# VladimirP1/rs-sync

Hardware: NVIDIA B200
Metric: presync_loss_evals_per_s (higher is better)
Workload: dtype f64

## Files before the change

### rs-sync_b200/csrc/engine.cu

```cuda
#include "engine.h"

#include <algorithm>
#include <atomic>
#include <cmath>
#include <cstdio>
#include <map>
#include <mutex>
#include <tuple>
#include <utility>
#include <vector>

#include "device_math.cuh"
#include "gyro_scan.h"

namespace rs {

namespace {

constexpr unsigned FULL = 0xffffffffu;

#ifdef RS_CHECKED
__device__ int* g_assert_slot = nullptr;
#define RS_ASSERT(cond)                                                      \
    do {                                                                     \
// ... 288 lines not shown
    return Vec3{M[0], M[1], M[2]};
}

template <int SLOTS>
__device__ __noinline__ unsigned long long warp_exact_quartile(const WarpSmem& w, int n, int lane,
                                                               double vx, double vy, double vz) {
    constexpr int NP = SLOTS * 32;
    const unsigned long long nanbits = 0x7ff8000000000000ULL;
    double r2[SLOTS];
    unsigned h[SLOTS];
    __syncwarp();
#pragma unroll
    for (int s = 0; s < SLOTS; ++s) {
        const int i = s * 32 + lane;
        const double p0 = w.P[i], p1 = w.P[NP + i], p2 = w.P[2 * NP + i];
        const double inv = (i < n) ? row_inv_norm(p0, p1, p2) : __longlong_as_double((long long)nanbits);
        const double r = dot3(p0 * inv, p1 * inv, p2 * inv, vx, vy, vz);
        r2[s] = r * r;
        h[s] = (unsigned)__double2hiint(r2[s]) & 0x7fffffffu;
    }
    const int kth = n / 4;
    int cl, ce;
    const unsigned H = warp_select_hi<SLOTS>(h, kth, 0x7ff80000u, lane, cl, ce);
    int rem = kth - cl;
    unsigned cur = 0u, lo_ans = 0u;
    for (;;) {
        unsigned mn = 0xffffffffu, c = 0u;
#pragma unroll
        for (int s = 0; s < SLOTS; ++s) {
            const unsigned lo = (unsigned)__double2loint(r2[s]);
            if (h[s] == H && lo >= cur) mn = min(mn, lo);
        }
        mn = __reduce_min_sync(FULL, mn);
#pragma unroll
        for (int s = 0; s < SLOTS; ++s)
            c += (h[s] == H && (unsigned)__double2loint(r2[s]) == mn) ? 1u : 0u;
        c = __reduce_add_sync(FULL, c);
        if (rem < (int)c) { lo_ans = mn; break; }
        rem -= (int)c;
        cur = mn + 1u;
    }
    return ((unsigned long long)H << 32) | lo_ans;
}

constexpr float kMargin = 1.4e-6f;

__device__ __forceinline__ unsigned up_bits(unsigned qbits) {
    const float u = __fadd_ru(__fsqrt_ru(__uint_as_float(qbits)), kMargin);
    return __float_as_uint(__fmul_ru(u, u));
}
__device__ __forceinline__ float sqrt_approx(float x) {
    float y;
    asm("sqrt.approx.ftz.f32 %0, %1;" : "=f"(y) : "f"(x));
    return y;
}

template <int SLOTS>
__device__ __forceinline__ int warp_count_le(const float (&s)[SLOTS], unsigned pv) {
    const float nt = -__uint_as_float(pv + 1u);
    unsigned c = 0;
#pragma unroll
    for (int i = 0; i < SLOTS; ++i) c += __float_as_uint(s[i] + nt) >> 31;
    return (int)__reduce_add_sync(FULL, c);
}
template <int SLOTS>
__device__ __forceinline__ unsigned warp_min_ge(const float (&s)[SLOTS], unsigned lo) {
    unsigned mn = 0xffffffffu;
#pragma unroll
    for (int i = 0; i < SLOTS; ++i) mn = min(mn, __float_as_uint(s[i]) - lo);
    return lo + __reduce_min_sync(FULL, mn);
}
template <int SLOTS>
__device__ __forceinline__ unsigned warp_max_lt(const float (&s)[SLOTS], unsigned hi_excl) {
    unsigned mn = 0xffffffffu;
    const unsigned top = hi_excl - 1u;
#pragma unroll
    for (int i = 0; i < SLOTS; ++i) mn = min(mn, top - __float_as_uint(s[i]));
    return top - __reduce_min_sync(FULL, mn);
}

template <int SLOTS>
__device__ __forceinline__ unsigned warp_select32(const float (&s)[SLOTS], int kk, unsigned hi_excl,
                                                  int chi, int npad, int n, bool sample) {
    unsigned lo = 0u;
    int clo = 0, poor = 0;
    for (int round = 0;; ++round) {
        RS_ASSERT(round < 80 && clo <= kk && kk < chi && lo < hi_excl);
        if (hi_excl - lo == 1u) return lo;
        if (kk == clo) return warp_min_ge<SLOTS>(s, lo);
        if (kk == chi - 1) return warp_max_lt<SLOTS>(s, hi_excl);
        unsigned pv;
        if (sample) {
            sample = false;
            const int js = min((32 * (kk - npad)) / n, 31);
            const unsigned k0 = __float_as_uint(s[0]);
            unsigned cur = 0u;
            pv = 0u;
            for (int i = 0; i <= js; ++i) {
                pv = cur + __reduce_min_sync(FULL, k0 - cur);
                cur = pv + 1u;
            }
        } else if (poor >= 2) {
            poor = 0;
            pv = lo + ((hi_excl - lo) >> 1);
        } else {
            const int cl = (lo == 0u) ? npad : clo;
            const float frac = ((float)(kk - cl) + 0.5f) / (float)(chi - cl);
            const float sl = sqrt_approx(__uint_as_float(lo));
            const float sh = sqrt_approx(__uint_as_float(hi_excl));
            const float sq = fmaf(sh - sl, frac, sl);
            pv = __float_as_uint(sq * sq);
        }
        pv = max(pv, lo);
        pv = min(pv, hi_excl - 2u);
        const int cnt = warp_count_le<SLOTS>(s, pv);
        if (cnt > kk) {
            poor = (2 * (cnt - clo) > (chi - clo)) ? poor + 1 : 0;
            hi_excl = pv + 1u;
            chi = cnt;
        } else {
            poor = (2 * (chi - cnt) > (chi - clo)) ? poor + 1 : 0;
            lo = pv + 1u;
            clo = cnt;
        }
    }
}

template <int SLOTS>
__device__ __forceinline__ bool load_normalised_rows32(const double* __restrict__ sP, int n, int lane,
                                                       float (&nx)[SLOTS], float (&ny)[SLOTS],
                                                       float (&nz)[SLOTS]) {
    constexpr int NP = SLOTS * 32;
    float fin = 0.f;
#pragma unroll
    for (int s = 0; s < SLOTS; ++s) {
        const int i = s * 32 + lane;
        const double r0 = sP[i], r1 = sP[NP + i], r2 = sP[2 * NP + i];
        const float n2 = (float)dot3(r0, r1, r2, r0, r1, r2);
        float rs;
        asm("rsqrt.approx.f32 %0, %1;" : "=f"(rs) : "f"(n2));
        if (i >= n) rs = 0.f;
        else if (n2 <= 1e-24f) rs = __uint_as_float(0x7fc00000u);
        nx[s] = (float)r0 * rs;
        ny[s] = (float)r1 * rs;
        nz[s] = (float)r2 * rs;
        fin += (fabsf(nx[s]) + fabsf(ny[s])) + fabsf(nz[s]);
    }
    return __all_sync(FULL, (__float_as_uint(fin) & 0x7f800000u) != 0x7f800000u);
}

enum FastStatus { kFastOk = 0, kFastUndecided = 1, kFastRowsNotFinite = 2, kFastRetry = 3 };

template <int SLOTS>
__device__ __forceinline__ FastStatus warp_ransac_fast(const DeviceData& dd, const FrameDesc& fd,
                                                       const WarpSmem& w, int iters, uint64_t key,
                                                       int lane, double M[3], int* settled,
                                                       unsigned prior, unsigned* tau_out) {
    constexpr int NP = SLOTS * 32;
    float nx[SLOTS], ny[SLOTS], nz[SLOTS];
    if (!load_normalised_rows32<SLOTS>(w.P, fd.n, lane, nx, ny, nz)) return kFastRowsNotFinite;
    const int n = fd.n;
    const int npad = NP - n;
    const int kk = n / 4 + npad;
    unsigned tau = 0x7f800000u;
    float nthr = 0.f;
    unsigned thr1 = 0u;
    bool has_real = true;
    if (prior) {
        tau = thr1 = prior;
        nthr = -__uint_as_float(prior);
        has_real = false;
    }
    M[0] = M[1] = M[2] = 0.0;
    float* hyp = w.hyp;
    for (int j0 = 0; j0 < iters; j0 += 32) {
        double v[3] = {0.0, 0.0, 0.0};
        if (j0 + lane < iters) draw_hypothesis(dd, fd, w.P, NP, key, (uint32_t)(j0 + lane), v);
        __syncwarp();
        hyp[lane] = (float)v[0];
        hyp[32 + lane] = (float)v[1];
        hyp[64 + lane] = (float)v[2];
        __syncwarp();
        const int cnt = (iters - j0) < 32 ? (iters - j0) : 32;
        int t = 0;
        while (t < cnt) {
            float sq[SLOTS];
            int tc, chi;
            unsigned hi_excl;
            bool first = false;
            if (tau == 0x7f800000u) {
                const float vx = hyp[t], vy = hyp[32 + t], vz = hyp[64 + t];
                unsigned mx = 0u;
#pragma unroll
                for (int s = 0; s < SLOTS; ++s) {
                    const float r = fmaf(nz[s], vz, fmaf(ny[s], vy, nx[s] * vx));
                    sq[s] = r * r;
                    mx = max(mx, __float_as_uint(sq[s]));
                }
                mx = __reduce_max_sync(FULL, mx);
                if (mx >= 0x7f800000u) return kFastUndecided;
                hi_excl = mx + 1u;
                chi = NP;
                tc = t;
                first = true;
                t += 1;
            } else {
                const int t1 = (t + 1 < cnt) ? t + 1 : t;
                const float2 vx2 = make_float2(hyp[t], hyp[t1]);
                const float2 vy2 = make_float2(hyp[32 + t], hyp[32 + t1]);
                const float2 vz2 = make_float2(hyp[64 + t], hyp[64 + t1]);
                const float2 nt2 = make_float2(nthr, nthr);
                float2 rr[SLOTS];
                unsigned c0 = 0, c1 = 0;
#pragma unroll
                for (int s = 0; s < SLOTS; ++s) {
                    float2 r = __fmul2_rn(vx2, make_float2(nx[s], nx[s]));
                    r = __ffma2_rn(vy2, make_float2(ny[s], ny[s]), r);
                    r = __ffma2_rn(vz2, make_float2(nz[s], nz[s]), r);
                    rr[s] = r;
                    const float2 e = __ffma2_rn(r, r, nt2);
                    c0 += __float_as_uint(e.x) >> 31;
                    c1 += __float_as_uint(e.y) >> 31;
                }
                const unsigned both = __reduce_add_sync(FULL, c0 | (c1 << 16));
                const int ca = (int)(both & 0xffffu), cb = (t1 != t) ? (int)(both >> 16) : 0;
                if (ca <= kk && cb <= kk) {
                    t += 2;
                    continue;
                }
                const bool second = ca <= kk;
                tc = second ? t1 : t;
                t += second ? 2 : 1;
                unsigned c = 0;
                const float nt = nthr;
#pragma unroll
                for (int s = 0; s < SLOTS; ++s) {
                    const float r = second ? rr[s].y : rr[s].x;
                    sq[s] = r * r;
                    c += __float_as_uint(sq[s] + nt) >> 31;
                }
                chi = (int)__reduce_add_sync(FULL, c);
                if (chi <= kk) continue;
                hi_excl = thr1;
            }
            const unsigned q = warp_select32<SLOTS>(sq, kk, hi_excl, chi, npad, n, first);
            const unsigned uq = up_bits(q);
            if (uq < tau) {
                tau = q;
                thr1 = uq + 1u;
                nthr = -__uint_as_float(thr1);
                has_real = true;
                M[0] = __shfl_sync(FULL, v[0], tc);
                M[1] = __shfl_sync(FULL, v[1], tc);
                M[2] = __shfl_sync(FULL, v[2], tc);
                continue;
            }
            if (!has_real) return kFastRetry;
            const double tx = __shfl_sync(FULL, v[0], tc), ty = __shfl_sync(FULL, v[1], tc),
                         tz = __shfl_sync(FULL, v[2], tc);
            const unsigned long long qt = warp_exact_quartile<SLOTS>(w, n, lane, tx, ty, tz);
            const unsigned long long qb = warp_exact_quartile<SLOTS>(w, n, lane, M[0], M[1], M[2]);
            if (qt >= 0x7ff0000000000000ULL || qb >= 0x7ff0000000000000ULL) return kFastUndecided;
            if (settled) ++*settled;
            if (qt < qb) {
                tau = q;
                thr1 = uq + 1u;
                nthr = -__uint_as_float(thr1);
                M[0] = tx; M[1] = ty; M[2] = tz;
            }
        }
    }
    if (!has_real) return kFastRetry;
    if (tau_out) *tau_out = tau;
    return kFastOk;
}

template <int SLOTS>
__device__ __forceinline__ unsigned warp_ransac(const DeviceData& dd, const FrameDesc& fd,
                                                const WarpSmem& w, int iters, uint64_t key, int lane,
                                                double M[3], unsigned* n_exact, unsigned prior = 0u,
                                                unsigned* tau_out = nullptr) {
    int settled = 0;
    FastStatus st = kFastRetry;
    unsigned tau = 0u;
    for (int attempt = 0; attempt < 2 && st == kFastRetry; ++attempt) {
        st = warp_ransac_fast<SLOTS>(dd, fd, w, iters, key, lane, M, &settled, attempt == 0 ? prior : 0u, &tau);
        if (!prior) break;
    }
    if (tau_out) *tau_out = (st == kFastOk) ? tau : 0u;
    if (n_exact && settled && lane == 0) atomicAdd(n_exact, 1u);
    if (st == kFastOk) return 0u;
    if (n_exact && !settled && lane == 0) atomicAdd(n_exact, 1u);
    const Vec3 e = warp_ransac_exact<SLOTS>(dd, fd, w, iters, key, lane);
    M[0] = e.x; M[1] = e.y; M[2] = e.z;
    return st == kFastRowsNotFinite ? kFlagP : 0u;
}

__device__ __noinline__ double warp_loss3_smem(const double* __restrict__ sP, int NP, int nslots,
                                               int lane, double m0, double m1, double m2, double k,
                                               const double* __restrict__ tab) {
    const double scale = k / sqrt(dot3(m0, m1, m2, m0, m1, m2));
    double acc = 0.0;
    for (int s = 0; s < nslots; ++s) {
        const int i = s * 32 + lane;
        const double r = dot3(sP[i], sP[NP + i], sP[2 * NP + i], m0, m1, m2) * scale;
        acc = acc + log1p_nonneg(r * r, tab);
    }
    return warp_sum(acc);
}

__device__ __noinline__ double warp_loss_rows_smem(const double* __restrict__ sP, int NP, int nslots,
                                                   int lane, double k, const double* __restrict__ tab) {
    double acc = 0.0;
    for (int s = 0; s < nslots; ++s) {
        const int i = s * 32 + lane;
        const double p0 = sP[i], p1 = sP[NP + i], p2 = sP[2 * NP + i];
        const double r = sqrt(dot3(p0, p1, p2, p0, p1, p2)) * k;
        acc = acc + log1p_nonneg(r * r, tab);
    }
    return warp_sum(acc);
}
__device__ __forceinline__ double warp_norm_rows(const double* sP, int NP, int nslots, int lane) {
    double ss = 0.0;
    for (int s = 0; s < nslots; ++s) {
        const int i = s * 32 + lane;
        const double p0 = sP[i], p1 = sP[NP + i], p2 = sP[2 * NP + i];
        const double nr = sqrt(dot3(p0, p1, p2, p0, p1, p2));
        ss = ss + nr * nr;
    }
    return sqrt(warp_sum(ss));
}

struct Loss5 {
    double f, g0, g1, g2;
};
__device__ __noinline__ Loss5 warp_loss5_smem(const double* __restrict__ sP, int NP, int nslots,
                                              int lane, double m0, double m1, double m2, double k,
                                              const double* __restrict__ tab) {
    const double kk = k * k;
    const double den = dot3(m0, m1, m2, m0, m1, m2) / kk;
    const double inv_den = 1.0 / den;
    double acc[5] = {0.0, 0.0, 0.0, 0.0, 0.0};
    for (int s = 0; s < nslots; ++s) {
        const int i = s * 32 + lane;
        const double p0 = sP[i], p1 = sP[NP + i], p2 = sP[2 * NP + i];
        const double v1 = dot3(p0, p1, p2, m0, m1, m2);
        const double u = (v1 * v1) * inv_den;
        acc[0] = acc[0] + log1p_nonneg(u, tab);
        const double wgt = 1.0 / (1.0 + u);
        const double wv = wgt * v1;
        acc[1] = acc[1] + wv * p0;
        acc[2] = acc[2] + wv * p1;
        acc[3] = acc[3] + wv * p2;
        acc[4] = acc[4] + wgt * u;
    }
    warp_sum_n<5>(acc);
    Loss5 out;
    out.f = acc[0];
    const double G0 = acc[1], G1 = acc[2], G2 = acc[3];
    const double SU = acc[4];
    const double c1 = 2.0 * inv_den;
    const double c2 = (c1 / kk) * SU;
    out.g0 = c1 * G0 - c2 * m0;
    out.g1 = c1 * G1 - c2 * m1;
    out.g2 = c1 * G2 - c2 * m2;
    return out;
}

template <int SLOTS>
__device__ __forceinline__ void load_rows(const double* __restrict__ sP, int NP, int lane,
                                          double (&p)[SLOTS][3]) {
#pragma unroll
    for (int s = 0; s < SLOTS; ++s) {
        const int i = s * 32 + lane;
        p[s][0] = sP[i];
        p[s][1] = sP[NP + i];
        p[s][2] = sP[2 * NP + i];
    }
}
template <int SLOTS>
__device__ __forceinline__ Loss5 warp_loss5_reg(const double (&p)[SLOTS][3], double m0, double m1,
                                                double m2, double k, const double* __restrict__ tab) {
    const double kk = k * k;
    const double den = dot3(m0, m1, m2, m0, m1, m2) / kk;
    const double inv_den = 1.0 / den;
    double v1[SLOTS], u[SLOTS], lg[SLOTS], wgt[SLOTS];
#pragma unroll
    for (int s = 0; s < SLOTS; ++s) {
        v1[s] = dot3(p[s][0], p[s][1], p[s][2], m0, m1, m2);
        u[s] = (v1[s] * v1[s]) * inv_den;
    }
#pragma unroll
    for (int s = 0; s < SLOTS; ++s) {
        lg[s] = log1p_nonneg(u[s], tab);
        wgt[s] = 1.0 / (1.0 + u[s]);
    }
    double r[5] = {0.0, 0.0, 0.0, 0.0, 0.0};
#pragma unroll
    for (int s = 0; s < SLOTS; ++s) {
        const double wv = wgt[s] * v1[s];
        r[0] = r[0] + lg[s];
        r[1] = r[1] + wv * p[s][0];
        r[2] = r[2] + wv * p[s][1];
        r[3] = r[3] + wv * p[s][2];
        r[4] = r[4] + wgt[s] * u[s];
    }
    warp_sum_n<5>(r);
    Loss5 out;
    out.f = r[0];
    const double c1 = 2.0 * inv_den;
    const double c2 = (c1 / kk) * r[4];
    out.g0 = c1 * r[1] - c2 * m0;
    out.g1 = c1 * r[2] - c2 * m1;
    out.g2 = c1 * r[3] - c2 * m2;
    return out;
}
template <int SLOTS>
__device__ __forceinline__ double warp_loss3_reg(const double (&p)[SLOTS][3], double m0, double m1,
                                                 double m2, double k, const double* __restrict__ tab) {
    const double scale = k / sqrt(dot3(m0, m1, m2, m0, m1, m2));
    double lg[SLOTS];
#pragma unroll
    for (int s = 0; s < SLOTS; ++s) {
        const double r = dot3(p[s][0], p[s][1], p[s][2], m0, m1, m2) * scale;
        lg[s] = log1p_nonneg(r * r, tab);
    }
    double acc = 0.0;
#pragma unroll
    for (int s = 0; s < SLOTS; ++s) acc = acc + lg[s];
    return warp_sum(acc);
}

constexpr int kLbfgsHistDoubles = 80;
template <class EvalF>
__device__ __forceinline__ double warp_lbfgs(EvalF&& eval, double x[3], int& n_iters, int& n_evals,
                                             double* __restrict__ hist) {
    constexpr int numBasis = 10, maxIterations = 200, maxTrials = 50;
    const double minGradientNorm = 1e-4, armijo = 1e-4, wolfe = 0.9, factr = 1e-15,
// ... 170 lines not shown
    int done_a[2];
    int next_task;
    int rec_first[2], rec_cnt[2];
    int frame[2], d0[2];
    int unit[2];
    FrameDesc fd[2];
};
static_assert(sizeof(GridCtl) <= 256, "GridCtl must fit its slot");

__device__ __noinline__ void grid_stage_unit(const DeviceData& dd, const FrameDesc* frames,
                                             const double* delays, int D, int chunk, int fi, int ci, int u,
                                             GridCtl* ctl, int b, double* sTiles, double* sRec, int rec_cap) {
    const int d0 = ci * chunk;
    const int d1 = min(D, d0 + chunk);
    const FrameDesc fd = frames[fi];
    double dmin = delays[d0], dmax = dmin;
    for (int d = d0 + 1; d < d1; ++d) {
        dmin = fmin(dmin, delays[d]);
        dmax = fmax(dmax, delays[d]);
    }
    const double x_lo = ((fd.ts_lo - dd.q0) + dmin) * dd.sr, x_hi = ((fd.ts_hi - dd.q0) + dmax) * dd.sr;
    const double r_lo = floor(x_lo) - 1.0, r_hi = floor(x_hi) + 2.0;
    const bool ok = dd.sr > 0.0 && r_lo >= 0.0 && r_hi <= (double)(dd.nq - 1) && (r_hi - r_lo) < (double)rec_cap;
    const int first = ok ? (int)r_lo : 0, cnt = ok ? (int)(r_hi - r_lo) + 1 : 0;
    ctl->rec_first[b] = first;
    ctl->rec_cnt[b] = cnt;
    ctl->frame[b] = fi;
    ctl->d0[b] = d0;
    ctl->fd[b] = fd;
    __threadfence_block();
    *(volatile int*)&ctl->unit[b] = u;
    asm volatile("fence.proxy.async.shared::cta;" ::: "memory");
    const unsigned tile_bytes = (unsigned)((fd.n + 31) >> 5) * 2048u;
    const unsigned bytes = ok ? (unsigned)cnt * 128u + tile_bytes : 0u;
    mbar_arrive_expect_tx(&ctl->full[b], bytes);
    if (ok) {
        tma_load_1d(sRec, dd.rec + (size_t)first * 16, (unsigned)cnt * 128u, &ctl->full[b]);
        tma_load_1d(sTiles, dd.rays + (size_t)fd.off * 8, tile_bytes, &ctl->full[b]);
    }
}

template <int SLOTS, bool SIMPLE>
__global__ void __launch_bounds__(GridCfg<SLOTS>::kWarps * 32, GridCfg<SLOTS>::kMinBlocks)
presync_kernel(DeviceData dd, const FrameDesc* __restrict__ frames, int F,
               const double* __restrict__ delays, int D, int chunk, int cpf, uint64_t seed,
               uint64_t stream, uint64_t call_no, const uint64_t* __restrict__ frame_call_no,
               uint64_t idx_base, double* __restrict__ framecost, int cost_stride,
               unsigned* __restrict__ flags, int staged) {
    using Cfg = GridCfg<SLOTS>;
    constexpr bool simplified = SIMPLE;
    extern __shared__ __align__(128) unsigned char smem_raw[];
    constexpr int NP = SLOTS * 32;
    const int lane = threadIdx.x & 31, warp = threadIdx.x >> 5;
    double* tab = reinterpret_cast<double*>(smem_raw);
    GridCtl* ctl = reinterpret_cast<GridCtl*>(smem_raw + Cfg::kCtlOff);
    unsigned char* bufs = smem_raw + Cfg::kBufOff;
    const WarpSmem w = warp_smem(smem_raw + Cfg::kWarpOff, warp, NP);
    const long long U = (long long)F * cpf;
    const long long u_begin = U * blockIdx.x / gridDim.x;
    const int n_units = (int)(U * (blockIdx.x + 1) / gridDim.x - u_begin);
    const int fi0 = (int)(u_begin / cpf), c0 = (int)(u_begin % cpf);
    auto stage = [&](int u) {
        const int cu = c0 + u, b = u & 1;
        double* sTiles = reinterpret_cast<double*>(bufs + (size_t)b * Cfg::kBufBytes);
        grid_stage_unit(dd, frames, delays, D, chunk, fi0 + cu / cpf, cu % cpf, u, ctl, b, sTiles,
                        sTiles + SLOTS * 256, Cfg::kRecs);
    };
    if (threadIdx.x == 0) {
        mbar_init(&ctl->full[0], 1);
        mbar_init(&ctl->full[1], 1);
        ctl->done_a[0] = ctl->done_a[1] = 0;
        ctl->unit[0] = ctl->unit[1] = -1;
        ctl->next_task = 0;
        asm volatile("fence.mbarrier_init.release.cluster;" ::: "memory");
    }
    load_log1p_table(tab);
    if (threadIdx.x == 0 && staged) {
        if (n_units > 0) stage(0);
        if (n_units > 1) stage(1);
    }
    const int n_tasks = n_units * chunk;
    int cur_u = -1, rec_first = 0, rec_cnt = 0, fi = 0, d0 = 0;
    FrameDesc fd{};
    unsigned prior = 0u;
    int prior_u = -1, prior_dj = -2;
    for (int k_next = 0, k_end = 0;;) {
        if (k_next == k_end) {
            if (lane == 0) k_next = atomicAdd(&ctl->next_task, RS_GRID_GRAB);
            k_next = __shfl_sync(FULL, k_next, 0);
            k_end = min(k_next + RS_GRID_GRAB, n_tasks);
            if (k_next >= n_tasks) break;
        }
        const int k = k_next++;
        const int u = k / chunk, dj = k - u * chunk;
        const int b = u & 1;
        if (u != cur_u && !staged) {
            cur_u = u;
            const int cu = c0 + u;
            fi = fi0 + cu / cpf;
            d0 = (cu % cpf) * chunk;
            fd = frames[fi];
        } else if (u != cur_u) {
            cur_u = u;
#ifdef RS_CHECKED
            unsigned spins = 0;
#endif
            for (int have; (have = *(volatile int*)&ctl->unit[b]) != u;) {
                RS_ASSERT(++spins < (1u << 24) && have < u);
                __nanosleep(RS_POLL_NS);
            }
            const unsigned parity = (unsigned)(u >> 1) & 1u;
            while (!mbar_try_wait(&ctl->full[b], parity)) {
                RS_ASSERT(++spins < (1u << 24));
                __nanosleep(RS_POLL_NS);
            }
            RS_ASSERT(*(volatile int*)&ctl->unit[b] == u);
            rec_first = *(volatile int*)&ctl->rec_first[b];
            rec_cnt = *(volatile int*)&ctl->rec_cnt[b];
            fi = *(volatile int*)&ctl->frame[b];
            d0 = *(volatile int*)&ctl->d0[b];
            const volatile FrameDesc* vf = &ctl->fd[b];
            fd.id = vf->id; fd.off = vf->off; fd.n = vf->n; fd.ts_lo = vf->ts_lo; fd.ts_hi = vf->ts_hi;
        }
        const int di = d0 + dj;
        const bool active = di < D;
        RS_ASSERT(fi >= 0 && fi < F && dj >= 0 && dj < chunk && fd.n >= 2 && fd.n <= NP);
        double delay = 0.0;
        if (active) {
            delay = delays[di];
            const double* sTiles = reinterpret_cast<const double*>(bufs + (size_t)b * Cfg::kBufBytes);
            if (rec_cnt) build_rows_staged(dd, fd, delay, lane, w, NP, sTiles, sTiles + SLOTS * 256, rec_first, rec_cnt);
            else build_rows_global_cold(dd, fd, delay, lane, w, NP);
        }
        __syncwarp();
        if (lane == 0 && staged) {
            __threadfence_block();
            RS_ASSERT(*(volatile int*)&ctl->unit[b] == u);
            const int done = atomicAdd(&ctl->done_a[b], 1);
            RS_ASSERT(done >= 0 && done < chunk);
            if (done == chunk - 1) {
                ctl->done_a[b] = 0;
                if (u + 2 < n_units) stage(u + 2);
            }
        }
        if (!active) continue;
        const uint64_t key =
            rng_task_key(rng_prefix(seed, stream, frame_call_no ? frame_call_no[fi] : call_no,
                                    idx_base + (uint64_t)di),
                         fd.id);
        double M[3] = {0.0, 0.0, 0.0};
        unsigned bad = 0u;
        if (!simplified) {
            const bool neighbour = RS_GRID_PRIOR && prior && prior_u == u && prior_dj + 1 == dj && prior < 0x7e000000u;
            unsigned tau = 0u;
            bad = warp_ransac<SLOTS>(dd, fd, w, 20, key, lane, M, flags + 1, neighbour ? prior + RS_PRIOR_BUMP : 0u,
                                     &tau);
            prior = tau;
            prior_u = u;
            prior_dj = dj;
        }
        __syncwarp();
        constexpr int LU = RS_LOSS_UNROLL < SLOTS ? RS_LOSS_UNROLL : SLOTS;
        double ss = 0.0;
#pragma unroll 1
        for (int s0 = 0; s0 < SLOTS; s0 += LU) {
            double pm[LU];
#pragma unroll
            for (int j = 0; j < LU; ++j) {
                const int i = (s0 + j) * 32 + lane;
                pm[j] = 0.0;
                if (s0 + j < SLOTS) {
                    const double p0 = w.P[i], p1 = w.P[NP + i], p2 = w.P[2 * NP + i];
                    pm[j] = simplified ? sqrt(dot3(p0, p1, p2, p0, p1, p2)) : dot3(p0, p1, p2, M[0], M[1], M[2]);
                    w.P[i] = pm[j];
                }
            }
#pragma unroll
            for (int j = 0; j < LU; ++j) ss = ss + pm[j] * pm[j];
        }
        const double kv = clamp_k(1.0 / sqrt(warp_sum(ss)) * 1e2);
        const double scale = simplified ? kv : kv / sqrt(dot3(M[0], M[1], M[2], M[0], M[1], M[2]));
        double acc = 0.0;
#pragma unroll 1
        for (int s0 = 0; s0 < SLOTS; s0 += LU) {
            double rho[LU];
#pragma unroll
            for (int j = 0; j < LU; ++j) {
                const double r = (s0 + j < SLOTS ? w.P[(s0 + j) * 32 + lane] : 0.0) * scale;
                rho[j] = sqrt(log1p_nonneg(r * r, tab));
            }
#pragma unroll
            for (int j = 0; j < LU; ++j) acc = acc + rho[j];
        }
        const double cost = sqrt(warp_sum(acc));
        if (lane == 0) framecost[(size_t)di * cost_stride + fi] = cost;
        if (bad || !is_finite(cost)) {
            bad = presync_diagnose(w.P, NP, (fd.n + 31) >> 5, lane, scale, M[0], M[1], M[2], tab);
            bad = __reduce_or_sync(FULL, bad);
            if (bad && lane == 0) atomicOr(flags, bad);
        }
    }
}

__global__ void reduce_rows_kernel(const double* __restrict__ in, int rows, int cols,
                                   double* __restrict__ out) {
    const int lane = threadIdx.x & 31;
    const int row = blockIdx.x * (blockDim.x >> 5) + (threadIdx.x >> 5);
    if (row >= rows) return;
    DD acc = dd_zero();
    for (int c = lane; c < cols; c += 32) dd_add(acc, in[(size_t)row * cols + c]);
    const double v = warp_dd_sum(acc);
    if (lane == 0) out[row] = v;
}

__global__ void reduce_windows_kernel(const double* __restrict__ in, int D, int F,
                                      const int* __restrict__ win_begin, int W,
                                      double* __restrict__ out) {
    const int lane = threadIdx.x & 31;
    const int q = blockIdx.x * (blockDim.x >> 5) + (threadIdx.x >> 5);
    if (q >= W * D) return;
    const int wi = q / D, d = q % D;
    DD acc = dd_zero();
    for (int f = win_begin[wi] + lane; f < win_begin[wi + 1]; f += 32) dd_add(acc, in[(size_t)d * F + f]);
    const double v = warp_dd_sum(acc);
    if (lane == 0) out[q] = v;
}

template <int SLOTS>
__global__ void __launch_bounds__(kWarpsPerBlock * 32)
sync_init_kernel(DeviceData dd, SyncBatchDev b, const double* __restrict__ sp_delay,
                 const uint64_t* __restrict__ sp_callno, const unsigned char* __restrict__ sp_active,
                 uint64_t seed) {
    extern __shared__ __align__(16) unsigned char smem_raw[];
    constexpr int NP = SLOTS * 32;
    const int lane = threadIdx.x & 31, warp = threadIdx.x >> 5;
    const WarpSmem w = warp_smem(smem_raw, warp, NP);
    for (int t = blockIdx.x * kWarpsPerBlock + warp; t < b.T; t += gridDim.x * kWarpsPerBlock) {
        const SyncTask task = b.tasks[t];
        if (!sp_active[task.sp]) continue;
        const int nslots = (task.fd.n + 31) >> 5;
        __syncwarp();
        build_rows_smem(dd, task.fd, sp_delay[task.sp], lane, w, NP);
        if (b.simplified) {
            const double nr = warp_norm_rows(w.P, NP, nslots, lane);
            if (lane == 0) {
                b.m[3 * t + 0] = 0.0; b.m[3 * t + 1] = 0.0; b.m[3 * t + 2] = 0.0;
                b.k[t] = clamp_k(1.0 / nr * 1e2);
            }
            continue;
        }
        const uint64_t key =
            rng_task_key(rng_prefix(seed, kStreamSyncInit, sp_callno[task.sp], 0), task.fd.id);
        double M[3];
        warp_ransac<SLOTS>(dd, task.fd, w, 200, key, lane, M, nullptr);
        __syncwarp();
        const double nrm = warp_norm_PM(w.P, NP, nslots, lane, M, nullptr);
        if (lane == 0) {
            b.m[3 * t + 0] = M[0]; b.m[3 * t + 1] = M[1]; b.m[3 * t + 2] = M[2];
            b.k[t] = clamp_k(1.0 / nrm * 1e2);
        }
    }
}

#ifndef RS_SYNC_MINB
#define RS_SYNC_MINB 1
#endif
template <bool SMALL>
struct LbfgsCfg {
    static constexpr int kWarps = SMALL ? 2 : kWarpsPerBlock;
    static constexpr int kMinBlocks = SMALL ? 6 : RS_SYNC_MINB;
};
template <int SLOTS, bool SMALL>
__global__ void __launch_bounds__(LbfgsCfg<SMALL>::kWarps * 32, SLOTS <= 8 ? LbfgsCfg<SMALL>::kMinBlocks : 1)
sync_motion_fgrad_kernel(DeviceData dd, SyncBatchDev b, const double* __restrict__ sp_delay,
                         const double* __restrict__ sp_x0,
                         const unsigned char* __restrict__ sp_active, double* __restrict__ scratch,
                         int* __restrict__ stats, unsigned long long* __restrict__ evals_total) {
    extern __shared__ __align__(16) unsigned char smem_raw[];
    constexpr int NP = SLOTS * 32;
    const int lane = threadIdx.x & 31, warp = threadIdx.x >> 5;
    double* tab = reinterpret_cast<double*>(smem_raw);
    load_log1p_table(tab);
    const WarpSmem w = warp_smem(smem_raw + kLog1pTableBytes, warp, NP);
    constexpr int W = LbfgsCfg<SMALL>::kWarps;
    double* hist = reinterpret_cast<double*>(smem_raw + kLog1pTableBytes + (size_t)W * warp_smem_bytes(NP)) +
                   warp * kLbfgsHistDoubles;
    for (int t = blockIdx.x * W + warp; t < b.T; t += gridDim.x * W) {
        const SyncTask task = b.tasks[t];
        if (!sp_active[task.sp]) continue;
        double m[3] = {b.m[3 * t], b.m[3 * t + 1], b.m[3 * t + 2]};
        const double k = b.k[t];
        const double x0 = sp_x0[task.sp];
        for (int j = b.simplified ? 1 : 0; j < 4; ++j) {
            const double delay = (j == 0)   ? sp_delay[task.sp]
                                 : (j == 1) ? x0
                                 : (j == 2) ? x0 - kNumericDiffStep
                                            : x0 + kNumericDiffStep;
            __syncwarp();
            build_rows_smem(dd, task.fd, delay, lane, w, NP);
            double p[SLOTS][3];
            load_rows<SLOTS>(w.P, NP, lane, p);
            if (j == 0) {
                int it, ev;
                warp_lbfgs([&](double a0, double a1, double a2) { return warp_loss5_reg<SLOTS>(p, a0, a1, a2, k, tab); },
                           m, it, ev, hist);
                if (lane == 0) {
// ... 805 lines not shown
                        double* d_f, int* d_stats, cudaStream_t st) {
    const int NP = slots_for(fd.n) * 32;
    probe_lbfgs_kernel<<<1, 32, kLog1pTableBytes + warp_smem_bytes(NP), st>>>(dd, fd, NP, delay, d_m, k, d_f, d_stats);
    g_launches += 1;
}
void launch_probe_guess(const DeviceData& dd, FrameDesc fd, double delay, int iters,
                        uint64_t key_prefix, int mode, double* d_mk, unsigned* d_n_exact,
                        cudaStream_t st) {
    RS_DISPATCH_SLOTS(fd.n, {
        auto kern = probe_guess_kernel<SL>;
        kern<<<1, 32, warp_smem_bytes(SL * 32), st>>>(dd, fd, delay, iters, key_prefix, mode,
                                                            d_mk, d_n_exact);
    });
    g_launches += 1;
}

void launch_ingest_pixels(const PixelFrame* d_frames, int n_frames, const double* d_points_a,
                          const double* d_points_b, LensDev lens, double image_rows, double* d_rays,
                          int32_t* d_orig, int32_t* d_pos, double* d_rowq, cudaStream_t st) {
    if (n_frames <= 0) return;
    ingest_pixels_kernel<<<n_frames, kIngestThreads, 0, st>>>(d_frames, d_points_a, d_points_b, lens,
                                                               image_rows, d_rays, d_orig, d_pos,
                                                               reinterpret_cast<double2*>(d_rowq));
    g_launches += 1;
}

void launch_retime_frames(const PixelFrame* d_frames, int n_frames, const double* d_src_rays,
                          const int32_t* d_src_orig, const double* d_rowq, double readout, double* d_rays,
                          int32_t* d_orig, int32_t* d_pos, double* d_ext, cudaStream_t st) {
    if (n_frames <= 0) return;
    retime_frames_kernel<<<n_frames, kIngestThreads, 0, st>>>(d_frames, d_src_rays, d_src_orig,
                                                               reinterpret_cast<const double2*>(d_rowq), readout,
                                                               d_rays, d_orig, d_pos,
                                                               reinterpret_cast<double4*>(d_ext));
    g_launches += 1;
}

void launch_ingest_rays(const PixelFrame* d_frames, int n_frames, const double* d_ts_a,
                        const double* d_ts_b, const double* d_rays_a, const double* d_rays_b,
                        double* d_rays, int32_t* d_orig, int32_t* d_pos, cudaStream_t st) {
    if (n_frames <= 0) return;
    ingest_rays_kernel<false><<<n_frames, kIngestThreads, 0, st>>>(d_frames, d_ts_a, d_ts_b, d_rays_a, d_rays_b,
                                                                    0.0, d_rays, d_orig, d_pos, nullptr);
    g_launches += 1;
}

void launch_ingest_row_fractions(const PixelFrame* d_frames, int n_frames, const double* d_frac_a,
                                 const double* d_frac_b, const double* d_rays_a, const double* d_rays_b,
                                 double readout, double* d_rays, int32_t* d_orig, int32_t* d_pos, double* d_rowq,
                                 cudaStream_t st) {
    if (n_frames <= 0) return;
    ingest_rays_kernel<true><<<n_frames, kIngestThreads, 0, st>>>(d_frames, d_frac_a, d_frac_b, d_rays_a, d_rays_b,
                                                                   readout, d_rays, d_orig, d_pos,
                                                                   reinterpret_cast<double2*>(d_rowq));
    g_launches += 1;
}

void launch_stage_rays(const int64_t* d_at, int n_frames, int64_t total, const double* rays_a,
                       const double* rays_b, const double* ts_a, const double* ts_b, double* d_stage,
                       StageInfo* d_info, cudaStream_t st) {
    if (n_frames <= 0) return;
    StageArgs a{d_at, total, {rays_a, rays_b, ts_a, ts_b},
                {d_stage + 2 * total, d_stage + 5 * total, d_stage, d_stage + total}, nullptr, 0.0, 1.0, d_info};
    stage_tracks_kernel<StageMode::kRays><<<n_frames, kStageThreads, 0, st>>>(a);
    g_launches += 1;
}

void launch_stage_row_fractions(const int64_t* d_at, const double* d_frame_ts, int n_frames, int64_t total,
                                const double* rays_a, const double* rays_b, const double* frac_a,
                                const double* frac_b, double readout, double* d_stage, StageInfo* d_info,
                                cudaStream_t st) {
    if (n_frames <= 0) return;
    StageArgs a{d_at, total, {rays_a, rays_b, frac_a, frac_b},
                {d_stage + 2 * total, d_stage + 5 * total, d_stage, d_stage + total}, d_frame_ts, readout, 1.0,
                d_info};
    stage_tracks_kernel<StageMode::kRowFractions><<<n_frames, kStageThreads, 0, st>>>(a);
    g_launches += 1;
}

void launch_stage_points(const int64_t* d_at, const double* d_frame_ts, int n_frames, int64_t total,
                         const double* points_a, const double* points_b, const LensDev& lens, double rows,
                         double* d_stage, StageInfo* d_info, cudaStream_t st) {
    if (n_frames <= 0) return;
    StageArgs a{d_at, total, {points_a, points_b, nullptr, nullptr}, {d_stage, d_stage + 2 * total, nullptr, nullptr},
                d_frame_ts, lens.ro, rows, d_info, lens.fx, lens.fy, lens.cx, lens.cy};
    stage_tracks_kernel<StageMode::kPoints><<<n_frames, kStageThreads, 0, st>>>(a);
    g_launches += 1;
}

void launch_spline_finish(const double* d_quats, const double* d_rhs, const double* d_diag, int n,
                          double* d_rec, cudaStream_t st) {
    if (n <= 0) return;
    const long long threads = 4LL * n;
    spline_finish_kernel<<<(unsigned)((threads + 255) / 256), 256, 0, st>>>(d_quats, d_rhs, d_diag, n, d_rec);
    g_launches += 1;
}

void launch_gyro_integrate(const double* d_ts, const double* d_gyro, int n, const double* h_matrices, int n_var,
                           void* d_orients, double* d_quats, double* d_prefix, cudaStream_t st) {
    if (n <= 0 || n_var <= 0) return;
    static_assert(sizeof(OrientDev) == 9 * sizeof(double), "OrientDev is one 3x3 matrix");
    cudaMemcpyAsync(d_orients, h_matrices, sizeof(OrientDev) * (size_t)n_var, cudaMemcpyHostToDevice, st);
    const int nb = (n + (int)kGyroScanBlock - 1) / (int)kGyroScanBlock;
    gyro_local_kernel<<<(nb * n_var + 31) / 32, 32, 0, st>>>(d_ts, d_gyro, n, static_cast<const OrientDev*>(d_orients), n_var, d_quats);
    gyro_prefix_kernel<<<(n_var + 31) / 32, 32, 0, st>>>(d_quats, n, n_var, d_prefix);
    const long long total = (long long)n * n_var;
    gyro_apply_kernel<<<(unsigned)((total + 255) / 256), 256, 0, st>>>(d_prefix, n, n_var, d_quats);
    g_launches += 3;
}
size_t gyro_orient_bytes(int n_var) { return sizeof(OrientDev) * (size_t)n_var; }
size_t gyro_prefix_doubles(int n, int n_var) {
    return (size_t)n_var * ((size_t)(n + (int)kGyroScanBlock - 1) / kGyroScanBlock + 1) * 4;
}

void launch_gyro_resample(const int64_t* d_ts_us, int count, const double* d_quats, int n_var, uint64_t tick0,
                          unsigned rate_hz, int n_out, double* d_out, unsigned* d_nonfinite, cudaStream_t st) {
    if (n_out <= 0 || n_var <= 0) return;
    const long long total = (long long)n_out * n_var;
    resample_kernel<<<(unsigned)((total + 127) / 128), 128, 0, st>>>(d_ts_us, count, d_quats, n_var, tick0, rate_hz, n_out,
                                                                     d_out, d_nonfinite);
    g_launches += 1;
}

void launch_spline_chains(const double* d_y, const double* d_f_down, const double* d_f_up, int n, int n_var,
                          double* d_rhs, cudaStream_t st) {
    if (n < 2 || n_var <= 0) return;
    spline_chains_kernel<<<(4 * n_var + 31) / 32, 32, 0, st>>>(d_y, d_f_down, d_f_up, n, n_var, d_rhs);
    g_launches += 1;
}

void launch_probe_trig(const double* d_x, int n, int which, double* d_out, cudaStream_t st) {
    probe_trig_kernel<<<(n + 255) / 256, 256, 0, st>>>(d_x, n, which, d_out);
    g_launches += 1;
}

float run_fp64_peak(int blocks, int threads, int iters, double* d_sink, cudaStream_t st) {
    cudaEvent_t e0, e1;
    cudaEventCreate(&e0);
    cudaEventCreate(&e1);
    fp64_peak_kernel<<<blocks, threads, 0, st>>>(iters / 8 + 1, d_sink);
    cudaEventRecord(e0, st);
    fp64_peak_kernel<<<blocks, threads, 0, st>>>(iters, d_sink);
    cudaEventRecord(e1, st);
    cudaEventSynchronize(e1);
    float ms = 0.f;
    cudaEventElapsedTime(&ms, e0, e1);
    cudaEventDestroy(e0);
    cudaEventDestroy(e1);
    g_launches += 2;
    return ms;
}

}
```

Measured before the change: 33.27 billion.

## Restructure RANSAC fast path with batched counting sweeps and bracketed threshold tightening

The sequential per-hypothesis scan in the fast RANSAC path is replaced by a batched sweep. Each sweep counts inliers for all 32 hypotheses in pairs and then processes the surviving candidates in order of count via a warp max-reduction. When no candidate is pending, a two-round interpolation bracket search tightens the threshold using an approximate quartile. That approximate threshold is later corrected with an exact select on the current best hypothesis. The aim is to cut the number of expensive warp_select32 and exact-quartile calls, at the cost of extra counting passes and more complex tie-breaking logic (a bidx index) that must match the reference ordering. Optional grid-statistics counters are added behind a compile flag.

Result: slower. 27.32 billion (median of 6 runs) (-17.9%).

```diff
diff --git a/rs-sync_b200/csrc/engine.cu b/rs-sync_b200/csrc/engine.cu
--- a/rs-sync_b200/csrc/engine.cu
+++ b/rs-sync_b200/csrc/engine.cu
@@ -464,6 +464,45 @@
 enum FastStatus { kFastOk = 0, kFastUndecided = 1, kFastRowsNotFinite = 2, kFastRetry = 3 };
 
 template <int SLOTS>
+__device__ __forceinline__ unsigned warp_count_pair(const float (&nx)[SLOTS], const float (&ny)[SLOTS],
+                                                    const float (&nz)[SLOTS], float2 vx2, float2 vy2,
+                                                    float2 vz2, float2 nt2) {
+    unsigned c0 = 0, c1 = 0;
+#pragma unroll
+    for (int s = 0; s < SLOTS; ++s) {
+        float2 r = __fmul2_rn(vx2, make_float2(nx[s], nx[s]));
+        r = __ffma2_rn(vy2, make_float2(ny[s], ny[s]), r);
+        r = __ffma2_rn(vz2, make_float2(nz[s], nz[s]), r);
+        const float2 e = __ffma2_rn(r, r, nt2);
+        c0 += __float_as_uint(e.x) >> 31;
+        c1 += __float_as_uint(e.y) >> 31;
+    }
+    return __reduce_add_sync(FULL, c0 | (c1 << 16));
+}
+template <int SLOTS>
+__device__ __forceinline__ void hyp_keys(const float (&nx)[SLOTS], const float (&ny)[SLOTS],
+                                         const float (&nz)[SLOTS], float vx, float vy, float vz,
+                                         float (&sq)[SLOTS]) {
+#pragma unroll
+    for (int s = 0; s < SLOTS; ++s) {
+        const float r = fmaf(nz[s], vz, fmaf(ny[s], vy, nx[s] * vx));
+        sq[s] = r * r;
+    }
+}
+__device__ __forceinline__ unsigned warp_top_candidate(int cl, int kk, int lane) {
+    return __reduce_max_sync(FULL, cl > kk ? ((unsigned)cl << 5) | (31u - lane) : 0u);
+}
+
+#ifdef RS_GRID_STATS
+enum GridStat { kStatTasks, kStatNoPrior, kStatRetries, kStatSelects, kStatBracketRounds, kStatBracketWins,
+                kStatRecounts, kStatSettles, kNumGridStats };
+__device__ unsigned long long g_grid_stats[kNumGridStats];
+#define RS_STAT(i) do { if ((threadIdx.x & 31) == 0) atomicAdd(&g_grid_stats[i], 1ull); } while (0)
+#else
+#define RS_STAT(i) do { } while (0)
+#endif
+
+template <int SLOTS>
 __device__ __forceinline__ FastStatus warp_ransac_fast(const DeviceData& dd, const FrameDesc& fd,
                                                        const WarpSmem& w, int iters, uint64_t key,
                                                        int lane, double M[3], int* settled,
@@ -475,12 +514,12 @@
     const int npad = NP - n;
     const int kk = n / 4 + npad;
     unsigned tau = 0x7f800000u;
-    float nthr = 0.f;
     unsigned thr1 = 0u;
     bool has_real = true;
+    bool exact = true;
+    int bidx = 0;
     if (prior) {
         tau = thr1 = prior;
-        nthr = -__uint_as_float(prior);
         has_real = false;
     }
     M[0] = M[1] = M[2] = 0.0;
@@ -494,90 +533,125 @@
         hyp[64 + lane] = (float)v[2];
         __syncwarp();
         const int cnt = (iters - j0) < 32 ? (iters - j0) : 32;
-        int t = 0;
-        while (t < cnt) {
+        const int t0 = (tau == 0x7f800000u) ? 1 : 0;
+        int cl = (t0 && lane == 0) ? kk + 1 : 0;
+        bool swept = false;
+        for (;;) {
+            unsigned top = warp_top_candidate(cl, kk, lane);
+            if (!top) {
+                if (swept) break;
+                swept = true;
+                const float nthr = -__uint_as_float(thr1);
+                const float2 nt2 = make_float2(nthr, nthr);
+                for (int t = t0; t < cnt; t += 2) {
+                    const int t1 = (t + 1 < cnt) ? t + 1 : t;
+                    const unsigned both = warp_count_pair<SLOTS>(nx, ny, nz, make_float2(hyp[t], hyp[t1]),
+                                                                 make_float2(hyp[32 + t], hyp[32 + t1]),
+                                                                 make_float2(hyp[64 + t], hyp[64 + t1]), nt2);
+                    if (lane == t) cl = (int)(both & 0xffffu);
+                    if (lane == t1 && t1 != t) cl = (int)(both >> 16);
+                }
+                top = warp_top_candidate(cl, kk, lane);
+                if (top && exact) {
+                    const int L = 31 - (int)(top & 31u);
+                    const float vx = hyp[L], vy = hyp[32 + L], vz = hyp[64 + L];
+                    unsigned lo = 0u, hi = thr1;
+                    int clo = npad, chi = (int)(top >> 5);
+#pragma unroll 1
+                    for (int round = 0; round < 2; ++round) {
+                        RS_STAT(kStatBracketRounds);
+                        const float frac = ((float)(kk - clo) + 0.5f) / (float)(chi - clo);
+                        const float sl = sqrt_approx(__uint_as_float(lo));
+                        const float sh = sqrt_approx(__uint_as_float(hi));
+                        const float e = fmaf(sh - sl, frac, sl);
+                        const float e1 = 0.95f * e, e2 = 1.05f * e;
+                        const unsigned p1 = min(max(__float_as_uint(e1 * e1), lo), hi);
+                        const unsigned p2 = min(max(__float_as_uint(e2 * e2), p1), hi);
+                        const unsigned both = warp_count_pair<SLOTS>(
+                            nx, ny, nz, make_float2(vx, vx), make_float2(vy, vy), make_float2(vz, vz),
+                            make_float2(-__uint_as_float(p1), -__uint_as_float(p2)));
+                        const int c1 = (int)(both & 0xffffu), c2 = (int)(both >> 16);
+                        if (c1 > kk) {
+                            hi = p1; chi = c1;
+                        } else if (c2 > kk) {
+                            lo = p1; clo = c1; hi = p2; chi = c2;
+                        } else {
+                            lo = p2; clo = c2;
+                        }
+                        if (lo != 0u && __uint_as_float(hi) <= 1.6f * __uint_as_float(lo)) break;
+                    }
+                    if (lo != 0u && __uint_as_float(hi) <= 1.6f * __uint_as_float(lo) && up_bits(hi) < tau) {
+                        RS_STAT(kStatBracketWins);
+                        tau = hi;
+                        thr1 = up_bits(hi) + 1u;
+                        exact = false;
+                        has_real = true;
+                        bidx = j0 + L;
+                        M[0] = __shfl_sync(FULL, v[0], L);
+                        M[1] = __shfl_sync(FULL, v[1], L);
+                        M[2] = __shfl_sync(FULL, v[2], L);
+                        if (lane == L) cl = 0;
+                    }
+                }
+                continue;
+            }
+            const int tc = 31 - (int)(top & 31u);
+            const bool first = tau == 0x7f800000u;
             float sq[SLOTS];
-            int tc, chi;
+            hyp_keys<SLOTS>(nx, ny, nz, hyp[tc], hyp[32 + tc], hyp[64 + tc], sq);
             unsigned hi_excl;
-            bool first = false;
-            if (tau == 0x7f800000u) {
-                const float vx = hyp[t], vy = hyp[32 + t], vz = hyp[64 + t];
+            int chi;
+            if (first) {
                 unsigned mx = 0u;
 #pragma unroll
-                for (int s = 0; s < SLOTS; ++s) {
-                    const float r = fmaf(nz[s], vz, fmaf(ny[s], vy, nx[s] * vx));
-                    sq[s] = r * r;
-                    mx = max(mx, __float_as_uint(sq[s]));
-                }
+                for (int s = 0; s < SLOTS; ++s) mx = max(mx, __float_as_uint(sq[s]));
                 mx = __reduce_max_sync(FULL, mx);
                 if (mx >= 0x7f800000u) return kFastUndecided;
                 hi_excl = mx + 1u;
                 chi = NP;
-                tc = t;
-                first = true;
-                t += 1;
             } else {
-                const int t1 = (t + 1 < cnt) ? t + 1 : t;
-                const float2 vx2 = make_float2(hyp[t], hyp[t1]);
-                const float2 vy2 = make_float2(hyp[32 + t], hyp[32 + t1]);
-                const float2 vz2 = make_float2(hyp[64 + t], hyp[64 + t1]);
-                const float2 nt2 = make_float2(nthr, nthr);
-                float2 rr[SLOTS];
-                unsigned c0 = 0, c1 = 0;
-#pragma unroll
-                for (int s = 0; s < SLOTS; ++s) {
-                    float2 r = __fmul2_rn(vx2, make_float2(nx[s], nx[s]));
-                    r = __ffma2_rn(vy2, make_float2(ny[s], ny[s]), r);
-                    r = __ffma2_rn(vz2, make_float2(nz[s], nz[s]), r);
-                    rr[s] = r;
-                    const float2 e = __ffma2_rn(r, r, nt2);
-                    c0 += __float_as_uint(e.x) >> 31;
-                    c1 += __float_as_uint(e.y) >> 31;
-                }
-                const unsigned both = __reduce_add_sync(FULL, c0 | (c1 << 16));
-                const int ca = (int)(both & 0xffffu), cb = (t1 != t) ? (int)(both >> 16) : 0;
-                if (ca <= kk && cb <= kk) {
-                    t += 2;
+                RS_STAT(kStatRecounts);
+                chi = warp_count_le<SLOTS>(sq, thr1 - 1u);
+                hi_excl = thr1;
+                if (chi <= kk) {
+                    if (lane == tc) cl = 0;
                     continue;
                 }
-                const bool second = ca <= kk;
-                tc = second ? t1 : t;
-                t += second ? 2 : 1;
-                unsigned c = 0;
-                const float nt = nthr;
-#pragma unroll
-                for (int s = 0; s < SLOTS; ++s) {
-                    const float r = second ? rr[s].y : rr[s].x;
-                    sq[s] = r * r;
-                    c += __float_as_uint(sq[s] + nt) >> 31;
-                }
-                chi = (int)__reduce_add_sync(FULL, c);
-                if (chi <= kk) continue;
-                hi_excl = thr1;
             }
+            const bool fix = !exact;
+            if (fix) {
+                hyp_keys<SLOTS>(nx, ny, nz, (float)M[0], (float)M[1], (float)M[2], sq);
+                hi_excl = tau + 1u;
+                chi = warp_count_le<SLOTS>(sq, tau);
+            } else if (lane == tc) {
+                cl = 0;
+            }
+            RS_STAT(kStatSelects);
             const unsigned q = warp_select32<SLOTS>(sq, kk, hi_excl, chi, npad, n, first);
             const unsigned uq = up_bits(q);
-            if (uq < tau) {
+            if (fix) {
                 tau = q;
                 thr1 = uq + 1u;
-                nthr = -__uint_as_float(thr1);
-                has_real = true;
-                M[0] = __shfl_sync(FULL, v[0], tc);
-                M[1] = __shfl_sync(FULL, v[1], tc);
-                M[2] = __shfl_sync(FULL, v[2], tc);
+                exact = true;
                 continue;
             }
-            if (!has_real) return kFastRetry;
             const double tx = __shfl_sync(FULL, v[0], tc), ty = __shfl_sync(FULL, v[1], tc),
                          tz = __shfl_sync(FULL, v[2], tc);
-            const unsigned long long qt = warp_exact_quartile<SLOTS>(w, n, lane, tx, ty, tz);
-            const unsigned long long qb = warp_exact_quartile<SLOTS>(w, n, lane, M[0], M[1], M[2]);
-            if (qt >= 0x7ff0000000000000ULL || qb >= 0x7ff0000000000000ULL) return kFastUndecided;
-            if (settled) ++*settled;
-            if (qt < qb) {
+            bool better = uq < tau;
+            if (!better) {
+                if (!has_real) return kFastRetry;
+                const unsigned long long qt = warp_exact_quartile<SLOTS>(w, n, lane, tx, ty, tz);
+                const unsigned long long qb = warp_exact_quartile<SLOTS>(w, n, lane, M[0], M[1], M[2]);
+                if (qt >= 0x7ff0000000000000ULL || qb >= 0x7ff0000000000000ULL) return kFastUndecided;
+                RS_STAT(kStatSettles);
+                if (settled) ++*settled;
+                better = qt < qb || (qt == qb && j0 + tc < bidx);
+            }
+            if (better) {
                 tau = q;
                 thr1 = uq + 1u;
-                nthr = -__uint_as_float(thr1);
+                has_real = true;
+                bidx = j0 + tc;
                 M[0] = tx; M[1] = ty; M[2] = tz;
             }
         }
@@ -596,6 +670,7 @@
     FastStatus st = kFastRetry;
     unsigned tau = 0u;
     for (int attempt = 0; attempt < 2 && st == kFastRetry; ++attempt) {
+        if (attempt) RS_STAT(kStatRetries);
         st = warp_ransac_fast<SLOTS>(dd, fd, w, iters, key, lane, M, &settled, attempt == 0 ? prior : 0u, &tau);
         if (!prior) break;
     }
@@ -1072,6 +1147,8 @@
         unsigned bad = 0u;
         if (!simplified) {
             const bool neighbour = RS_GRID_PRIOR && prior && prior_u == u && prior_dj + 1 == dj && prior < 0x7e000000u;
+            RS_STAT(kStatTasks);
+            if (!neighbour) RS_STAT(kStatNoPrior);
             unsigned tau = 0u;
             bad = warp_ransac<SLOTS>(dd, fd, w, 20, key, lane, M, flags + 1, neighbour ? prior + RS_PRIOR_BUMP : 0u,
                                      &tau);
@@ -2183,3 +2260,14 @@
 }
 
 }
+
+#ifdef RS_GRID_STATS
+extern "C" int rssync_grid_stats(unsigned long long* out, int n) {
+    if (n < rs::kNumGridStats) return -1;
+    if (cudaDeviceSynchronize() != cudaSuccess) return -2;
+    if (cudaMemcpyFromSymbol(out, rs::g_grid_stats, sizeof(rs::g_grid_stats)) != cudaSuccess) return -2;
+    const unsigned long long zero[rs::kNumGridStats] = {};
+    if (cudaMemcpyToSymbol(rs::g_grid_stats, zero, sizeof(zero)) != cudaSuccess) return -2;
+    return rs::kNumGridStats;
+}
+#endif
```
